# jorgeMFS/VCFX

Hardware: AMD Instinct MI355X
Metric: variant-records/sec (and GB/s vs HBM roofline), 427K var × 2504 samp (higher is better)
Workload: dtype u8; 1 GPU; VCFX_allele_freq_calc -i (file path) on a device-resident 427409 x 2504 VCF shard per GPU: the walk (line ends + allele counts + rows composed in LDS) + the rows in file order; records_per_gpu=427409, samples=2504, bytes_per_gpu=4297544426, parallelism=record-sharded x1

## Files before the change

### vcfx_amd/csrc/gpu/vcfxg_af_walk.hip

```cpp
#include <algorithm>
#include <type_traits>

#include "vcfxg_device.h"
#include "vcfxg_gt.h"
#include "vcfxg_kernels.h"
#include "vcfxg_walk.h"

namespace vcfxg {

#ifndef VCFXG_WALK_UNROLL
#define VCFXG_WALK_UNROLL 6
#endif
constexpr int kWalkUnroll = VCFXG_WALK_UNROLL;
#ifndef VCFXG_HWE_UNROLL
#define VCFXG_HWE_UNROLL 5
#endif
constexpr int kHweUnroll = VCFXG_HWE_UNROLL;
#ifndef VCFXG_GF_FLAGS
#define VCFXG_GF_FLAGS 1
#endif
constexpr bool kGfFlags = VCFXG_GF_FLAGS != 0;
#ifndef VCFXG_GF_UNROLL
#define VCFXG_GF_UNROLL 4
#endif
constexpr int kGfUnroll = VCFXG_GF_UNROLL;
#ifndef VCFXG_AF_XREC
#define VCFXG_AF_XREC 0
#endif
#ifndef VCFXG_AF_EXPT
#define VCFXG_AF_EXPT 0
#endif
#ifndef VCFXG_AF_EARLY
#define VCFXG_AF_EARLY 0
#endif
#define VCFXG_STR2(x) #x
#define VCFXG_STR(x) VCFXG_STR2(x)

template <class Op>
struct WalkRed;
template <>
struct WalkRed<AfOp> {
    static constexpr bool kAux = false;
    __device__ static AfOp make(const char *buf, int64_t ae) { return AfOp{buf, ae, 0}; }
    __device__ static void out(const AfOp &op, uint32_t &a, uint32_t &b, uint32_t &) {
        a = op.alt;
        b = op.tot;
    }
};
template <>
struct WalkRed<HweOp> {
    static constexpr bool kAux = true;
    __device__ static HweOp make(const char *buf, int64_t ae) { return HweOp{buf, ae}; }
    __device__ static void out(const HweOp &op, uint32_t &a, uint32_t &b, uint32_t &c) {
        a = op.c0;
        b = op.c1;
        c = op.c2;
    }
};

template <>
struct WalkRed<DoseWalkOp> {
    static constexpr bool kAux = false;
    __device__ static DoseWalkOp make(const char *buf, int64_t ae) { return DoseWalkOp{buf, ae}; }
    __device__ static void out(const DoseWalkOp &op, uint32_t &a, uint32_t &b, uint32_t &) {
        a = op.ns;
        b = op.na;
    }
};

template <>
struct WalkRed<DoseHeadOp> : WalkRed<DoseWalkOp> {
    __device__ static DoseHeadOp make(const char *buf, int64_t ae) { return DoseHeadOp{{buf, ae}}; }
};

template <class Op, bool kGF = false>
__global__ __launch_bounds__(kWalkThreads)
#ifdef VCFXG_WALK_MAXW
__attribute__((amdgpu_waves_per_eu(1, VCFXG_WALK_MAXW)))
#else
#ifndef VCFXG_AF_MINW
#define VCFXG_AF_MINW 5
#endif
__attribute__((amdgpu_waves_per_eu(kGF ? 4 : VCFXG_AF_MINW)))
#endif
void k_af_walk(const char *__restrict__ buf, int64_t lo, int64_t hi, int64_t chunk, int64_t n_walkers, int mode,
               int64_t span0, uint64_t cap_w, uint64_t *__restrict__ le_o, int32_t *__restrict__ alt_o,
               int32_t *__restrict__ tot_o, int32_t *__restrict__ aux_o, uint32_t *__restrict__ rowpre_o,
               uint8_t *__restrict__ status_o, LineMeta *__restrict__ meta_o, uint64_t *__restrict__ wcount,
               uint32_t *__restrict__ wgt, unsigned *overflow, WalkTail tail) {
    typedef WalkRed<Op> R;
    __shared__ uint4 win[kWalkWaves][2][kWave];
    constexpr bool kStageLds = std::is_same<Op, AfOp>::value;
    constexpr uint32_t kStgCap = kStageLds ? 2048u : 16u;
    __shared__ __attribute__((aligned(16))) char stg[kStageLds ? kWalkWaves : 1][kStgCap];
    const int wv = threadIdx.x / kWave;
    const int64_t wk = uniform64((int64_t)walk_block() * kWalkWaves + wv);
    if (wk >= n_walkers) return;
    const int strip_cr = mode == 0 ? 1 : 0;
    const int64_t cs = lo + wk * chunk;
    const int64_t ce = std::min<int64_t>(cs + chunk, hi);
    int64_t L, ce2;
    walker_lines(buf, lo, hi, cs, ce, L, ce2, chunk);
    const int64_t L0 = L;
    uint64_t wtext = 0;
    int64_t span = span0;
    uint8_t cr_prev = 0;
    uint64_t n = 0;
    uint32_t ngt = 0, ngf = 0;
    bool dirty = false;
    const uint64_t base = (uint64_t)wk * cap_w;
    uint64_t r_le = 0, r_S = 0;
    uint32_t r_alt = 0, r_tot = 0, r_aux = 0, r_pre = 0, r_k = 0;
    uint32_t r_h = 0;
    auto flush = [&](uint64_t first, uint32_t cnt) {
        if ((uint32_t)lane() < cnt) {
            const uint64_t o = base + first + lane();
            const uint8_t kind = (uint8_t)r_k;
            LineMeta m{};
            m.kind = kind;
            m.cr = (uint8_t)(r_k >> 16);
            m.pad = (R::kAux || std::is_same<Op, DoseHeadOp>::value) ? (uint8_t)r_h : 0;
            if (kind == kMetaGt) {
                m.S = r_S;
                m.rowpre = r_pre;
                m.sep = (uint8_t)(r_k >> 8);
            }
            le_o[o] = r_le;
            alt_o[o] = (int32_t)r_alt;
            tot_o[o] = (int32_t)r_tot;
            if (R::kAux) aux_o[o] = (int32_t)r_aux;
            rowpre_o[o] = kind == kMetaGt ? r_pre : 0u;
            status_o[o] = (uint8_t)(r_k >> 24);
            meta_o[o] = m;
        }
    };
    constexpr bool kXrec = VCFXG_AF_XREC && std::is_same<Op, AfOp>::value && !kGF;
    uint4 xv[kXrec ? kWalkUnroll : 1];
    int64_t xvb = -1;
    int cur = 0;
    int64_t A = L & ~(int64_t)15;
    if (L < ce2) prefetch_window(buf, A, hi, win[wv][cur]);
    constexpr bool kEarly = VCFXG_AF_EARLY && std::is_same<Op, AfOp>::value && !kGF && !kXrec;
    uint4 ev[kEarly ? kWalkUnroll : 1];
    const int64_t hlast = (hi - 1) & ~(int64_t)15;
    while (L < ce2) {
        if (n >= cap_w) {
            if (lane() == 0) atomicOr(overflow, 1u);
            break;
        }
        if constexpr (kEarly) {
#pragma unroll
            for (int u = 0; u < kWalkUnroll; u++) {
                const int64_t g = A + u * kWaveStep + kBlockBytes * lane();
                ev[u] = load16(buf, g < hi ? g : hlast);
            }
        }
        int64_t eA = kEarly ? A : -1;
        const int Lr = (int)(L - A);
        const uint4 *cw = win[wv][cur];
        int hr, N1r, r4 = 0, r7 = 0, r8 = 0;
        uint32_t ntab, first, hflags = 0;
        auto take = [&](const int(&rt)[9], bool comma) {
            r4 = rt[4];
            r7 = rt[7];
            r8 = rt[8];
            if (R::kAux) {
                const bool empty = rt[0] == Lr || rt[1] == rt[0] + 1 || r4 == rt[3] + 1;
                hflags = (comma ? kHweAltComma : 0u) | (empty ? kHweEmptyField : 0u);
            }
        };
        uint32_t w4 = 0;
        bool long_head = false;
        {
            if constexpr (kEarly) asm volatile("s_waitcnt vmcnt(" VCFXG_STR(VCFXG_WALK_UNROLL) ")" ::: "memory");
            else asm volatile("s_waitcnt vmcnt(0)" ::: "memory");
            w4 = reinterpret_cast<const uint32_t *>(cw)[lane()];
            hr = (int)std::min<int64_t>(hi - A, kWin);
            const uint32_t rg = range4(Lr, hr);
            N1r = first_match<4>(zero_bytes(w4 ^ kRepNl) & rg);
            int rt[9] = {};
            ntab = first_tabs<4>(zero_bytes(w4 ^ kRepTab) & rg, N1r >= 0 ? N1r : hr, rt);
            first = dword_byte(w4, Lr);
            if (ntab >= 9) take(rt, R::kAux && __ballot((zero_bytes(w4 ^ 0x2C2C2C2Cu) & range4(rt[3] + 1, rt[4])) != 0u));
        }
        if (N1r < 0 && ntab < 9 && first != '#' && hr == kWin) {
            prefetch_window(buf, A, hi, win[wv][cur], kWaveStep);
            long_head = true;
            const uint4 W = read_window(cw);
            const int b = 16 * lane();
            hr = (int)std::min<int64_t>(hi - A, kWaveStep);
            N1r = first_match<16>(eq_mask16(W, kRepNl) & range16(b, Lr, hr));
            int rt[9] = {};
            ntab = first_tabs<16>(eq_mask16(W, kRepTab) & range16(b, Lr, hr), N1r >= 0 ? N1r : hr, rt);
            if (ntab >= 9) take(rt, R::kAux && __ballot((eq_mask16(W, 0x2C2C2C2Cu) & range16(b, rt[3] + 1, rt[4])) != 0u));
        }
        auto wbyte = [&](int o) { return long_head ? slot_byte(cw, o) : dword_byte(w4, o); };
        const int64_t wend = A + hr;
        int64_t t4 = -1, t8 = -1;
        bool gt_head = false, gt_only = false;
        if (ntab >= 9 && first != '#') {
            t4 = A + r4;
            t8 = A + r8;
            if (r8 - r7 >= 3 && wbyte(r7 + 1) == 'G' && wbyte(r7 + 2) == 'T') {
                gt_only = r8 - r7 == 3;
                gt_head = gt_only || wbyte(r7 + 3) == ':';
            }
        }
        int64_t E;
        uint8_t cr = 0;
        bool predicted = false;
        const bool gf = kGF && N1r < 0 && gt_head && !gt_only;
        if (N1r >= 0) {
            E = A + N1r;
            cr = strip_cr && E > L && wbyte(N1r - 1) == '\r';
        } else if (gf) {
            E = hi;
        } else if (gt_only && span > 0 && t8 + 1 + span <= hi) {
            E = t8 + 1 + span;
            cr = cr_prev;
            predicted = true;
        } else {
            E = scan_nl(buf, wend, hi);
            cr = strip_cr && E > L && __builtin_amdgcn_readfirstlane(byte_at(buf, E - 1)) == '\r';
        }
        const uint32_t sep_w = gt_head && t8 + 2 < wend ? wbyte((int)(t8 + 2 - A)) : 0u;
        const int nxt = cur ^ 1;
        int64_t An = std::max<int64_t>(E - 1, 0) & ~(int64_t)15;
        bool pending = true;
        auto pre = [&]() {
            prefetch_window(buf, An, hi, win[wv][nxt]);
            pending = false;
        };
        uint8_t st = 0, kind = 0, sep = 0;
        uint32_t alt = 0, tot = 0, aux = 0, rowpre = 0;
        int64_t S = 0;
        bool ok = false;
        bool skip = std::is_same<Op, DoseHeadOp>::value && predicted;
        int64_t xuse = xvb;
        xvb = -1;
        auto sweep = [&]() {
            if constexpr (kGF) {
              if (gf) {
                S = t8 + 1;
                Op op = R::make(buf, hi);
                int64_t Eo = hi;
                uint8_t cro = 0;
                auto pre_e = [&](int64_t e) {
                    An = std::max<int64_t>(e - 1, 0) & ~(int64_t)15;
                    pre();
                };
                if constexpr (std::is_same<Op, AfOp>::value && kGfFlags)
                    ok = gt_first_af<kGfUnroll>(buf, S, hi, strip_cr, op, pre_e, Eo, cro);
                else
                    ok = gt_first<kWalkUnroll>(buf, S, hi, strip_cr, op, pre_e, Eo, cro);
                E = Eo;
                cr = cro;
                const int64_t ae = E - cr;
                kind = t8 < ae ? kMetaGt : kMetaFull;
                ok = ok && kind == kMetaGt;
                if (kind == kMetaGt) {
                    rowpre = (uint32_t)(t4 - L + 1);
                    sep = t8 + 2 >= ae ? 0
                          : t8 + 2 < wend ? (uint8_t)sep_w
                                          : (uint8_t)__builtin_amdgcn_readfirstlane(byte_at(buf, t8 + 2));
                    R::out(op, alt, tot, aux);
                }
                return;
              }
            }
            const int64_t ae = E - cr;
            if (ae <= L) kind = kMetaEmpty;
            else if (first == '#') kind = kMetaHeader;
            else if (gt_head && t8 < ae) kind = kMetaGt;
            else kind = kMetaFull;
            ok = false;
            if (kind == kMetaGt) {
                S = t8 + 1;
                rowpre = (uint32_t)(t4 - L + 1);
                sep = t8 + 2 >= ae ? 0
                      : t8 + 2 < wend ? (uint8_t)sep_w
                                      : (uint8_t)__builtin_amdgcn_readfirstlane(byte_at(buf, t8 + 2));
                Op op = R::make(buf, ae);
                if constexpr (kXrec) {
                    const int64_t use = xuse >= 0 && xuse <= S ? xuse : -1;
                    xuse = -1;
                    const int64_t nb = E + 1 < ce2 ? (E + 1) & ~(int64_t)15 : -1;
                    int64_t vbo;
                    ok = af_fixed_x<kWalkUnroll>(buf, S, ae, hi, op, sep, pre, xv, use, nb, vbo);
                    xvb = vbo;
                } else if constexpr (kEarly) {
                    const bool mine = eA >= 0 && eA <= S;
                    ok = af_fixed<kWalkUnroll>(buf, S, ae, op, sep, pre, mine ? ev : nullptr, mine ? eA : -1);
                    eA = -1;
                } else if constexpr (std::is_same<Op, AfOp>::value)
                    ok = af_fixed < kGF ? kGfUnroll : kWalkUnroll > (buf, S, ae, op, sep, pre);
                else if constexpr (std::is_same<Op, DoseHeadOp>::value) {
                    if (skip) {
                        ok = (sep == '/' || sep == '|') && ae - S >= 3 && ((ae - S + 1) & 3) == 0;
                        op.ns = ok ? (uint32_t)((ae - S + 1) >> 2) : 0u;
                        op.na = 0;
                    } else {
                        ok = gt_fast<kWalkUnroll>(buf, S, ae, op, sep, pre);
                    }
                } else ok = gt_fast < std::is_same<Op, HweOp>::value ? kHweUnroll : kWalkUnroll > (buf, S, ae, op, sep, pre);
                R::out(op, alt, tot, aux);
            }
        };
        sweep();
        if (pending) pre();
        if (predicted) {
            const uint4 *nw = win[wv][nxt];
            asm volatile("s_waitcnt vmcnt(0)" ::: "memory");
            const uint32_t be = slot_byte(nw, (int)(E - An)), be1 = slot_byte(nw, (int)(E - 1 - An));
            const bool endok = (E < hi ? be == '\n' : true) && ((strip_cr && be1 == '\r') == (cr != 0));
            if (!(ok && endok)) {
                const int64_t Et = scan_nl(buf, wend, hi);
                if (Et != E || !endok) {
                    skip = false;
                    E = Et;
                    cr = strip_cr && E > L && __builtin_amdgcn_readfirstlane(byte_at(buf, E - 1)) == '\r';
                    An = std::max<int64_t>(E - 1, 0) & ~(int64_t)15;
                    pending = true;
                    sweep();
                    if (pending) pre();
                }
            }
        }
        if constexpr (std::is_same<Op, DoseHeadOp>::value)
            if (skip && kind == kMetaGt) hflags |= kWalkUnswept;
        if (kind == kMetaGt) {
            if (ok) {
                st = 1;
                span = E - S;
                cr_prev = cr;
            } else {
                st = kAfPending;
            }
        }
        if ((uint32_t)lane() == (uint32_t)(n & 63)) {
            r_le = (uint64_t)E;
            r_S = (uint64_t)S;
            r_alt = alt;
            r_tot = tot;
            r_aux = aux;
            r_h = hflags;
            r_pre = rowpre;
            r_k = (uint32_t)kind | ((uint32_t)sep << 8) | ((uint32_t)cr << 16) | ((uint32_t)st << 24);
        }
        if constexpr (std::is_same<Op, AfOp>::value) {
            if (tail.stage && !(VCFXG_AF_EXPT & 1)) {
                if (kind == kMetaGt && ok && wtext + rowpre + 7u <= std::min<uint32_t>(tail.stage_cap, kStgCap)) {
                    uint32_t flo = 0x30303030u, fhi = 0x0A3030u;
                    if (!(VCFXG_AF_EXPT & 2)) af_freq_text(mode, (int32_t)alt, (int32_t)tot, flo, fhi);
                    auto *dst = reinterpret_cast<__attribute__((address_space(3))) char *>(
                                    reinterpret_cast<__attribute__((address_space(3))) char *>(
                                        (__attribute__((address_space(3))) void *)stg[kStageLds ? wv : 0])) +
                                wtext;
                    const unsigned char *src = reinterpret_cast<const unsigned char *>(cw) + (L - A);
                    for (uint32_t j0 = 0; j0 < rowpre + 7u; j0 += kWave) {
                        const uint32_t j = j0 + (uint32_t)lane();
                        if (j < rowpre) dst[j] = (char)src[j];
                        else if (j < rowpre + 7u) {
                            const uint32_t q = j - rowpre;
                            dst[j] = (char)((q < 4u ? flo >> (8u * q) : fhi >> (8u * (q - 4u))) & 0xFFu);
                        }
                    }
                } else if (kind == kMetaGt || kind == kMetaFull) {
                    dirty = true;
                }
            }
        }
        ngt += kind == kMetaGt ? 1u : 0u;
        if constexpr (kGF) ngf += gf && kind == kMetaGt && ok ? 1u : 0u;
        if (tail.wtext) {
            if (kind == kMetaGt) wtext += (uint64_t)rowpre + 7u;
            if (kind == kMetaFull || (kind == kMetaGt && !ok)) {
                if (lane() == 0) {
                    const unsigned long long e = atomicAdd(tail.cx_n, 1ull);
                    if (e < tail.cx_cap) tail.cx_list[e] = base + n;
                }
            }
        }
        n++;
        if ((n & 63) == 0) flush(n - 64, 64);
        L = E + 1;
        A = An;
        cur = nxt;
    }
    if (n & 63) flush(n & ~(uint64_t)63, (uint32_t)(n & 63));
    if constexpr (kStageLds) {
        if (tail.stage && wtext) {
            __builtin_amdgcn_fence(__ATOMIC_RELEASE, "wavefront");
            __builtin_amdgcn_wave_barrier();
            __builtin_amdgcn_fence(__ATOMIC_ACQUIRE, "wavefront");
            const uint32_t wt = (uint32_t)std::min<uint64_t>(wtext, kStgCap);
            char *gs = tail.stage + (uint64_t)wk * tail.stage_cap;
            for (uint32_t o = (uint32_t)lane() * 16u; o < wt; o += kWave * 16u)
                *reinterpret_cast<uint4 *>(gs + o) = *reinterpret_cast<const uint4 *>(stg[wv] + o);
        }
    }
    if (lane() == 0) {
        wcount[wk] = n;
        if (tail.wtext) {
            tail.wtext[wk] = wtext;
            tail.wstart[wk] = (uint64_t)L0;
        }
        wgt[wk] = ngt | (ngf << 16);
        if (tail.wdirty) tail.wdirty[wk] = dirty || n >= cap_w ? 1 : 0;
    }
}

#ifndef VCFXG_COMPACT_SUB
#define VCFXG_COMPACT_SUB 4
#endif
constexpr int kCompactSub = VCFXG_COMPACT_SUB, kCompactLanes = kWave / kCompactSub;
__global__ __launch_bounds__(256) void k_walk_compact(int64_t n_walkers, uint64_t cap_w,
                                                      const uint64_t *__restrict__ offs,
                                                      const uint32_t *__restrict__ wgt,
                                                      const uint64_t *__restrict__ le_b,
                                                      const int32_t *__restrict__ alt_b,
                                                      const int32_t *__restrict__ tot_b,
                                                      const int32_t *__restrict__ aux_b,
                                                      const uint32_t *__restrict__ rowpre_b,
                                                      const uint8_t *__restrict__ status_b,
                                                      const LineMeta *__restrict__ meta_b, uint64_t *line_end,
                                                      int32_t *alt, int32_t *tot, int32_t *aux, uint32_t *rowpre,
                                                      uint8_t *status, LineMeta *meta, uint64_t *n_lines,
                                                      unsigned long long *counters, const uint64_t *__restrict__ bpre) {
    __shared__ uint32_t red[256 / kWave];
    uint32_t g = 0;
    const int64_t nwaves = (int64_t)gridDim.x * (256 / kWave);
    const int sub = lane() / kCompactLanes, sl = lane() % kCompactLanes;
    for (int64_t w0 = ((int64_t)blockIdx.x * (256 / kWave) + threadIdx.x / kWave) * kCompactSub; w0 < n_walkers;
         w0 += nwaves * kCompactSub) {
        const int64_t w = w0 + sub;
        if (w >= n_walkers) continue;
        const uint64_t d0 = offs[w] + (bpre ? bpre[w / kWalkerScanBlock] : 0),
                       cnt = offs[w + 1] + (bpre ? bpre[(w + 1) / kWalkerScanBlock] : 0) - d0, s0 = (uint64_t)w * cap_w;
        g += sl == 0 ? (wgt[w] & 0xFFFFu) : 0u;
        for (uint64_t i = sl; i < cnt; i += kCompactLanes) {
            const uint64_t sl = s0 + i, d = d0 + i;
            line_end[d] = le_b[sl];
            alt[d] = alt_b[sl];
            tot[d] = tot_b[sl];
            if (aux_b) aux[d] = aux_b[sl];
            rowpre[d] = rowpre_b[sl];
            status[d] = status_b[sl];
            meta[d] = meta_b[sl];
        }
    }
    g = wave_sum(g);
    if (lane() == 0) red[threadIdx.x / kWave] = g;
    __syncthreads();
    if (threadIdx.x == 0) {
        uint32_t t = 0;
        for (int k = 0; k < 256 / kWave; k++) t += red[k];
        if (t) {
            atomicAdd(&counters[0], (unsigned long long)t);
            atomicAdd(&counters[1], (unsigned long long)t);
        }
        if (blockIdx.x == 0) *n_lines = offs[n_walkers] + (bpre ? bpre[n_walkers / kWalkerScanBlock] : 0);
    }
}

int64_t af_walkers(int64_t lo, int64_t hi, int64_t chunk) { return hi > lo ? (hi - lo + chunk - 1) / chunk : 0; }

hipError_t launch_af_walk(const char *buf, int64_t lo, int64_t hi, int64_t chunk, int mode, int64_t span0,
                          uint64_t cap_w, uint64_t *le_b, int32_t *alt_b, int32_t *tot_b, uint32_t *rowpre_b,
                          uint8_t *status_b, void *meta_b, uint64_t *wcount, uint32_t *wgt, unsigned *overflow,
                          hipStream_t s, int32_t *hwe_aux_b, const WalkTail *tail, bool dose, bool gt_first_walk,
                          bool dose_head) {
    const WalkTail t = tail ? *tail : WalkTail{};
    const int64_t nw = af_walkers(lo, hi, chunk);
    if (!nw) return hipErrorInvalidValue;
    const unsigned grid = (unsigned)((nw + kWalkWaves - 1) / kWalkWaves);
    if (gt_first_walk)
        hipLaunchKernelGGL(HIP_KERNEL_NAME(k_af_walk<AfOp, true>), dim3(grid), dim3(kWalkThreads), 0, s, buf, lo, hi,
                           chunk, nw, mode, span0, cap_w, le_b, alt_b, tot_b, nullptr, rowpre_b, status_b,
                           static_cast<LineMeta *>(meta_b), wcount, wgt, overflow, t);
    else if (dose && dose_head)
        hipLaunchKernelGGL(k_af_walk<DoseHeadOp>, dim3(grid), dim3(kWalkThreads), 0, s, buf, lo, hi, chunk, nw, mode,
                           span0, cap_w, le_b, alt_b, tot_b, nullptr, rowpre_b, status_b, static_cast<LineMeta *>(meta_b),
                           wcount, wgt, overflow, t);
    else if (dose)
        hipLaunchKernelGGL(k_af_walk<DoseWalkOp>, dim3(grid), dim3(kWalkThreads), 0, s, buf, lo, hi, chunk, nw, mode,
                           span0, cap_w, le_b, alt_b, tot_b, nullptr, rowpre_b, status_b, static_cast<LineMeta *>(meta_b),
                           wcount, wgt, overflow, t);
    else if (hwe_aux_b)
        hipLaunchKernelGGL(k_af_walk<HweOp>, dim3(grid), dim3(kWalkThreads), 0, s, buf, lo, hi, chunk, nw, mode, span0,
                           cap_w, le_b, alt_b, tot_b, hwe_aux_b, rowpre_b, status_b, static_cast<LineMeta *>(meta_b),
                           wcount, wgt, overflow, t);
    else
        hipLaunchKernelGGL(k_af_walk<AfOp>, dim3(grid), dim3(kWalkThreads), 0, s, buf, lo, hi, chunk, nw, mode, span0,
                           cap_w, le_b, alt_b, tot_b, nullptr, rowpre_b, status_b, static_cast<LineMeta *>(meta_b),
                           wcount, wgt, overflow, t);
    return hipGetLastError();
}

hipError_t launch_walk_compact(int64_t n_walkers, uint64_t cap_w, const uint64_t *offs, const uint32_t *wgt,
                               const uint64_t *le_b, const int32_t *alt_b, const int32_t *tot_b,
                               const uint32_t *rowpre_b, const uint8_t *status_b, const void *meta_b,
                               uint64_t *line_end, int32_t *alt, int32_t *tot, uint32_t *rowpre, uint8_t *status,
                               void *meta, uint64_t *n_lines, unsigned long long *counters, hipStream_t s,
                               const int32_t *aux_b, int32_t *aux, const uint64_t *bpre) {
    const int64_t blocks = std::min<int64_t>((n_walkers + 256 / kWave - 1) / (256 / kWave), 512);
    hipLaunchKernelGGL(k_walk_compact, dim3((unsigned)std::max<int64_t>(blocks, 1)), dim3(256), 0, s, n_walkers, cap_w,
                       offs, wgt, le_b, alt_b, tot_b, aux_b, rowpre_b, status_b, static_cast<const LineMeta *>(meta_b),
                       line_end, alt, tot, aux, rowpre, status, static_cast<LineMeta *>(meta), n_lines, counters, bpre);
    return hipGetLastError();
}

}
```

### vcfx_amd/csrc/gpu/vcfxg_gt.h

```cpp
#pragma once
#include <algorithm>
#include <type_traits>

#include "vcfxg_device.h"

#ifndef VCFXG_AF_ROLL
#define VCFXG_AF_ROLL 0
#endif
#ifndef VCFXG_GF_BUF
#define VCFXG_GF_BUF 1
#endif

#ifndef VCFXG_FQ_EXPT
#define VCFXG_FQ_EXPT 0
#endif

namespace vcfxg {

struct DwordView {
    uint32_t d;
    uint32_t f;
    uint32_t dig;
    bool real;
    int64_t p;
};

template <class Op>
__device__ __forceinline__ void fast_dword(uint32_t d, uint32_t exp_xor, uint32_t &err, Op &op, bool real,
                                           int64_t p) {
    uint32_t e = d ^ exp_xor;
    err |= e & 0xFF00FF00u;
    uint32_t f = e & 0x00FF00FFu;
    uint32_t notdig = (f + 0x00F600F6u) & 0x01000100u;
    uint32_t notdot = ((f ^ 0x001E001Eu) + 0x00FF00FFu) & 0x01000100u;
    err |= notdig & notdot;
    DwordView v{d, f, notdig ^ 0x01000100u, real, p};
    op.dword(v);
}

#ifndef VCFXG_UNROLL
#define VCFXG_UNROLL 4
#endif
#ifndef VCFXG_NT_SWEEP
#define VCFXG_NT_SWEEP 0
#endif
struct NoPre {
    __device__ void operator()() const {}
};
template <class T, class = void>
struct HasClean : std::false_type {};
template <class T>
struct HasClean<T, std::void_t<decltype(&T::clean)>> : std::true_type {};
template <class T, class = void>
struct HasCleanAt : std::false_type {};
template <class T>
struct HasCleanAt<T, std::void_t<decltype(&T::clean_at)>> : std::true_type {};
template <int kUnroll = VCFXG_UNROLL, class Op, class Pre = NoPre>
__device__ bool gt_fast(const char *__restrict__ buf, int64_t S, int64_t E, Op &op, uint32_t sep_hint = 0,
                        Pre pre = Pre(), int64_t *swept = nullptr) {
    S = uniform64(S);
    E = uniform64(E);
    int64_t L = E - S;
    if (L < 3 || ((L + 1) & 3)) return false;
    uint32_t sepc = sep_hint ? sep_hint : byte_at(buf, S + 1);
    sepc = __builtin_amdgcn_readfirstlane(sepc);
    if (sepc != '/' && sepc != '|') return false;
    const uint32_t exp_xor = 0x09000000u | (sepc << 8) | 0x00300030u;
    const uint32_t neutral = 0x092E002Eu | (sepc << 8);
    op.begin(sepc, neutral);
    const int s = (int)(S & 3);
    const int64_t b0 = S & ~(int64_t)15;
    const char *__restrict__ base = buf + b0;
    const int Sr = (int)(S - b0), Er = (int)(E - b0);
#if VCFXG_NT_SWEEP
    const int lastblk = (Er - 1) & ~15;
#endif
    uint32_t err = 0;
    if (swept) *swept = E;
    const int lo16 = lane() * kBlockBytes;
#if !VCFXG_NT_SWEEP
    const __amdgpu_buffer_rsrc_t rs = buf_rsrc(base, (uint32_t)((Er + 15) & ~15));
#endif
    for (int w0 = 0; w0 < Er; w0 += kUnroll * kWaveStep) {
        uint4 v[kUnroll];
        uint32_t x4[kUnroll];
#pragma unroll
        for (int u = 0; u < kUnroll; u++) {
            const int blk = w0 + u * kWaveStep + lo16;
#if VCFXG_NT_SWEEP
            const int bl = blk < Er ? blk : lastblk;
            {
                typedef unsigned int v4u __attribute__((ext_vector_type(4)));
                const v4u t = __builtin_nontemporal_load(reinterpret_cast<const v4u *>(base + bl));
                v[u] = make_uint4(t.x, t.y, t.z, t.w);
            }
            x4[u] = load4(base, bl + 16);
#else
            v[u] = bload16(rs, blk);
            x4[u] = bload4(rs, blk + 16);
#endif
        }
        if (w0 == 0) pre();
#pragma unroll
        for (int u = 0; u < kUnroll; u++) {
            const int w = w0 + u * kWaveStep;
            const int blk = w + lo16;
            const bool interior = (w + s >= Sr) && (w + kWaveStep - 1 + s < Er);
            if (blk < Er) {
                uint32_t d[4] = {__builtin_amdgcn_alignbyte(v[u].y, v[u].x, s),
                                 __builtin_amdgcn_alignbyte(v[u].z, v[u].y, s),
                                 __builtin_amdgcn_alignbyte(v[u].w, v[u].z, s),
                                 __builtin_amdgcn_alignbyte(x4[u], v[u].w, s)};
                bool clean = false;
                if constexpr (HasClean<Op>::value || HasCleanAt<Op>::value) {
                    if (interior) {
                        const uint32_t e0 = d[0] ^ exp_xor, e1 = d[1] ^ exp_xor, e2 = d[2] ^ exp_xor,
                                       e3 = d[3] ^ exp_xor;
                        clean = !__any(((e0 | e1 | e2 | e3) & ~0x00010001u) != 0u);
                        if (clean) {
                            if constexpr (HasCleanAt<Op>::value) op.clean_at(e0, e1, e2, e3, b0 + blk + s);
                            else op.clean(e0, e1, e2, e3);
                        }
                    }
                }
                bool real[4] = {true, true, true, true};
                if (!interior) {
                    const int q0 = blk + s - Sr, last = Er - Sr - 3;
#pragma unroll
                    for (int i = 0; i < 4; i++) {
                        const int q = q0 + 4 * i;
                        if (q < 0 || q > last) {
                            d[i] = neutral;
                            real[i] = false;
                        } else if (q == last) d[i] = (d[i] & 0x00FFFFFFu) | 0x09000000u;
                    }
                }
                if (!clean) {
#pragma unroll
                    for (int i = 0; i < 4; i++) fast_dword(d[i], exp_xor, err, op, real[i], b0 + blk + s + 4 * i);
                }
            }
        }
        if (op.done()) {
            if (swept && b0 + w0 + kUnroll * kWaveStep < E) *swept = b0 + w0 + kUnroll * kWaveStep;
            break;
        }
        if (__any(err != 0u)) return false;
    }
    if (__any(err != 0u)) return false;
    op.finish();
    return true;
}

template <class Op>
__device__ void gt_general(const char *__restrict__ buf, int64_t S, int64_t E, Op &op) {
    for (int64_t w = S & ~(int64_t)15; w < E; w += kWaveStep) {
        int64_t blk = w + (int64_t)lane() * kBlockBytes;
        if (blk < E) {
            uint32_t tm = eq_mask16(load16(buf, blk), kRepTab);
            uint32_t starts = (tm << 1) & 0xFFFFu;
            if (blk > 0 && byte_at(buf, blk - 1) == '\t') starts |= 1u;
            starts &= range_mask16(blk, S + 1, E);
            if (S >= blk && S < blk + 16) starts |= 1u << (S - blk);
            while (starts) {
                int j = __builtin_ctz(starts);
                starts &= starts - 1u;
                op.sample(blk + j);
            }
        }
        if (op.done()) break;
    }
    op.finish();
}

__device__ __forceinline__ int64_t sample_end(const char *__restrict__ buf, int64_t st, int64_t E) {
    int64_t p = st;
    while (p < E && byte_at(buf, p) != '\t') p++;
    return p;
}

__device__ __forceinline__ bool gt_special(uint32_t c) {
    return c == '/' || c == '|' || c == ':' || c == '\t' || c == ' ' || c == '\r';
}
template <int kU, class Op, class Pre>
__device__ bool gt_first(const char *__restrict__ buf, int64_t S, int64_t hi, int strip_cr, Op &op, Pre pre,
                         int64_t &E_out, uint8_t &cr_out) {
    S = uniform64(S);
    int64_t E = hi, ae = hi;
    bool found = false, bad = false;
    uint32_t carry = 0;
    const int64_t b0 = S & ~(int64_t)15;
    const int lo16 = lane() * kBlockBytes;
    for (int64_t w0 = b0; w0 < hi && !found; w0 += kU * kWaveStep) {
        uint4 v[kU];
        uint32_t x4[kU];
#pragma unroll
        for (int u = 0; u < kU; u++) {
            const int64_t blk = w0 + u * kWaveStep + lo16;
            const int64_t bl = blk < hi ? blk : ((hi - 1) & ~(int64_t)15);
            v[u] = load16(buf, bl);
            x4[u] = load4(buf, bl + 16);
        }
#pragma unroll
        for (int u = 0; u < kU; u++) {
            if (found) break;
            const int64_t blk = w0 + u * kWaveStep + lo16;
            const uint32_t nlm = blk < hi ? eq_mask16(v[u], kRepNl) & range_mask16(blk, S, hi) : 0u;
            const uint64_t anyn = __ballot(nlm != 0u);
            if (anyn) {
                const int k = __builtin_ctzll(anyn);
                E = uniform64(w0 + u * kWaveStep + 16 * k + __builtin_ctz((uint32_t)__shfl((int)nlm, k)));
                found = true;
                const uint32_t cr = strip_cr && E > S ? __builtin_amdgcn_readfirstlane(byte_at(buf, E - 1)) == '\r' : 0u;
                cr_out = (uint8_t)cr;
                ae = E - cr;
                pre(E);
            }
            const uint32_t tm = eq_mask16(v[u], kRepTab);
            const uint32_t last = lane_prev(v[u].w >> 24);
            const uint32_t prev = lane() ? last : carry;
            carry = lane_last(v[u].w >> 24);
            uint32_t starts = ((tm << 1) & 0xFFFFu) | (prev == '\t' ? 1u : 0u);
            if (S >= blk && S < blk + 16) starts |= 1u << (S - blk);
            starts &= range_mask16(blk, S, ae);
            const uint32_t wd[5] = {v[u].x, v[u].y, v[u].z, v[u].w, x4[u]};
            while (starts) {
                const int o = __builtin_ctz(starts);
                starts &= starts - 1u;
                const int q = o >> 2;
                const uint32_t lo = q == 0 ? wd[0] : q == 1 ? wd[1] : q == 2 ? wd[2] : wd[3];
                const uint32_t hw = q == 0 ? wd[1] : q == 1 ? wd[2] : q == 2 ? wd[3] : wd[4];
                const uint32_t d = __builtin_amdgcn_alignbyte(hw, lo, (uint32_t)(o & 3));
                const uint32_t c0 = d & 0xFFu, c1 = (d >> 8) & 0xFFu, c2 = (d >> 16) & 0xFFu, c3 = d >> 24;
                const int64_t p3 = blk + o + 3;
                const bool quick = (c1 == '/' || c1 == '|') && !gt_special(c0) && !gt_special(c2) &&
                                   (p3 == ae || (p3 < ae && (c3 == ':' || c3 == '\t')));
                if (quick) op.gt3(c0, c2);
                else bad = true;
            }
        }
    }
    if (!found) {
        E = hi;
        const uint32_t cr = strip_cr && E > S ? __builtin_amdgcn_readfirstlane(byte_at(buf, E - 1)) == '\r' : 0u;
        cr_out = (uint8_t)cr;
        pre(E);
    }
    E_out = E;
    if (__any(bad)) return false;
    op.finish();
    return true;
}
struct NoPreE {
    __device__ void operator()(int64_t) const {}
};
template <int kU = 8, class Op>
__device__ __forceinline__ bool gt_first_known(const char *__restrict__ buf, int64_t S, int64_t ae, Op &op) {
    int64_t e;
    uint8_t cr;
    return gt_first<kU>(buf, S, ae, 0, op, NoPreE(), e, cr);
}

struct AfOp {
    const char *buf;
    int64_t E;
    int gi;
    uint32_t alt = 0, tot = 0;
    __device__ void begin(uint32_t, uint32_t) {}
    __device__ bool done() const { return false; }
    __device__ void dword(const DwordView &v) {
        tot += __popc(v.dig);
        alt += __popc((v.f + 0x00FF00FFu) & v.dig);
    }
    __device__ void gt3(uint32_t c0, uint32_t c2) {
        tot += (c0 - '0' < 10u) + (c2 - '0' < 10u);
        alt += (c0 - '1' < 9u) + (c2 - '1' < 9u);
    }
    __device__ void sample(int64_t st) {
        int64_t p = st;
        for (int k = 0; k < gi; k++) {
            while (p < E) {
                uint32_t c = byte_at(buf, p);
                if (c == '\t' || c == ':') break;
                p++;
            }
            if (p >= E || byte_at(buf, p) == '\t') return;
            p++;
        }
        bool in_tok = false, first_dot = false, numeric = true, nonzero = false;
        for (;; p++) {
            uint32_t c = p < E ? byte_at(buf, p) : (uint32_t)'\t';
            bool end = (c == '\t' || c == ':');
            if (end || c == '/' || c == '|') {
                if (in_tok && !first_dot && numeric) {
                    tot++;
                    if (nonzero) alt++;
                }
                in_tok = false;
                if (end) break;
                continue;
            }
            if (!in_tok) {
                in_tok = true;
                first_dot = (c == '.');
                numeric = true;
                nonzero = false;
            }
            if (c < '0' || c > '9') numeric = false;
            else if (c != '0') nonzero = true;
        }
    }
    __device__ void finish() {
        alt = wave_sum(alt);
        tot = wave_sum(tot);
    }
};

__device__ __forceinline__ uint32_t fixed4_mmap(double v) {
    double sc = __dadd_rn(__dmul_rn(v, 10000.0), 0.5);
    return (uint32_t)(unsigned long long)sc;
}
__device__ __forceinline__ uint32_t fixed4_printf(double v) {
    if (v == 0.0) return 0u;
    uint64_t bits = __double_as_longlong(v);
    int ex = (int)((bits >> 52) & 0x7FF);
    uint64_t m = bits & ((1ull << 52) - 1);
    int q;
    if (ex == 0) q = 1074;
    else { m |= 1ull << 52; q = 1075 - ex; }
    if (q <= 0) return 10000u * (uint32_t)(m << -q);
    unsigned __int128 num = (unsigned __int128)m * 10000u;
    if (q >= 100) return 0u;
    unsigned __int128 k = num >> q;
    unsigned __int128 rem = num - (k << q);
    unsigned __int128 half = (unsigned __int128)1 << (q - 1);
    if (rem > half || (rem == half && (k & 1))) k += 1;
    return (uint32_t)k;
}

__device__ __forceinline__ void af_freq_text(int mode, int32_t a, int32_t t, uint32_t &lo, uint32_t &hi) {
    const double f = t > 0 ? __ddiv_rn((double)a, (double)t) : 0.0;
    const uint32_t k4 = mode == 0 ? fixed4_mmap(f) : fixed4_printf(f);
    const uint32_t ip = k4 / 10000u, fp = k4 % 10000u;
    lo = ('0' + ip) | ((uint32_t)'.' << 8) | (('0' + fp / 1000u) << 16) | (('0' + (fp / 100u) % 10u) << 24);
    hi = ('0' + (fp / 10u) % 10u) | (('0' + fp % 10u) << 8) | ((uint32_t)'\n' << 16);
}
template <int kU, class Pre>
__device__ bool gt_first_af(const char *__restrict__ buf, int64_t S, int64_t hi, int strip_cr, AfOp &op, Pre pre,
                            int64_t &E_out, uint8_t &cr_out) {
    S = uniform64(S);
    constexpr uint32_t M = 0x80808080u, K = 0x7F7F7F7Fu;
    int64_t E = hi, ae = hi;
    bool found = false;
    uint32_t bad = 0, asc = 0, tot = 0, alt = 0;
    uint32_t carry = 0;
    uint32_t scarry = 0;
    const int64_t b0 = S & ~(int64_t)15;
    const int lo16 = lane() * kBlockBytes;
    const int64_t hend = (hi + 15) & ~(int64_t)15;
    for (int64_t w0 = b0; w0 < hi && !found; w0 += kU * kWaveStep) {
        uint4 v[kU];
        uint32_t x4[kU];
#if VCFXG_GF_BUF
        const __amdgpu_buffer_rsrc_t rs =
            buf_rsrc(buf + w0, (uint32_t)std::min<int64_t>(hend - w0, (int64_t)kU * kWaveStep + 16));
#pragma unroll
        for (int u = 0; u < kU; u++) {
            v[u] = bload16(rs, u * kWaveStep + lo16);
            x4[u] = bload4(rs, u * kWaveStep + lo16 + 16);
        }
#else
#pragma unroll
        for (int u = 0; u < kU; u++) {
            const int64_t blk = w0 + u * kWaveStep + lo16;
            const int64_t bl = blk < hi ? blk : hend - 16;
            v[u] = load16(buf, bl);
            x4[u] = load4(buf, bl + 16);
        }
#endif
#pragma unroll
        for (int u = 0; u < kU; u++) {
            if (found) break;
            const int64_t ws = w0 + u * kWaveStep, blk = ws + lo16;
            const uint32_t W[5] = {v[u].x, v[u].y, v[u].z, v[u].w, x4[u]};
            const uint32_t wor = W[0] | W[1] | W[2] | W[3];
            asc |= wor | W[4];
            const bool first = ws == b0, edge = first || ws + kWaveStep > hi;
            uint32_t nlm = 0;
            if (edge) nlm = blk < hi ? eq_mask16(v[u], kRepNl) & range_mask16(blk, S, hi) : 0u;
            else
                nlm = (~(((W[0] ^ kRepNl) + K) & ((W[1] ^ kRepNl) + K) & ((W[2] ^ kRepNl) + K) &
                         ((W[3] ^ kRepNl) + K)) | wor) & M;
            uint64_t anyn = __ballot(nlm != 0u);
            if (anyn && !edge) {
                nlm = eq_mask16(v[u], kRepNl);
                anyn = __ballot(nlm != 0u);
            }
            if (anyn) {
                const int k = __builtin_ctzll(anyn);
                E = uniform64(ws + 16 * k + __builtin_ctz((uint32_t)__shfl((int)nlm, k)));
                found = true;
                const uint32_t cr = strip_cr && E > S ? __builtin_amdgcn_readfirstlane(byte_at(buf, E - 1)) == '\r' : 0u;
                cr_out = (uint8_t)cr;
                ae = E - cr;
                pre(E);
            }
            const uint32_t tab3 = ~((W[3] ^ kRepTab) + K);
            const uint32_t up = lane_prev(tab3);
            uint32_t tprev = lane() ? up : carry;
            carry = lane_last(tab3);
            uint32_t rm = 0xFFFFu;
            if (edge || found) {
                rm = blk < hi ? range_mask16(blk, S, ae) : 0u;
                rm |= ((S >= blk && S < blk + 16) ? 1u << (S - blk) : 0u) << 16;
            }
            uint32_t st[4];
            {
                uint32_t tp = tprev;
#pragma unroll
                for (int i = 0; i < 4; i++) {
                    const uint32_t tb = i == 3 ? tab3 : ~((W[i] ^ kRepTab) + K);
                    uint32_t x = __builtin_amdgcn_alignbyte(tb, tp, 3) & M;
                    if (edge || found)
                        x = (x | nib_bytes((rm >> (16 + 4 * i)) & 0xFu)) & nib_bytes((rm >> (4 * i)) & 0xFu) & M;
                    st[i] = x;
                    tp = tb;
                }
            }
            const uint32_t sup = lane_prev(st[3]);
            const uint32_t sprev = lane() ? sup : scarry;
            scarry = lane_last(st[3]);
            auto classes = [&](uint32_t x, uint32_t &sep, uint32_t &trm, uint32_t &vv, uint32_t &dg, uint32_t &nz) {
                const uint32_t nt = (x ^ kRepTab) + K, nn = (x ^ kRepNl) + K, nc = (x ^ kRepColon) + K;
                trm = ~(nt & nn & nc);
                const uint32_t ns = (x ^ 0x2F2F2F2Fu) + K;
                sep = ~(ns & ((x ^ 0x7C7C7C7Cu) + K));
                const uint32_t g9 = x + 0x46464646u;
                dg = (x + 0x50505050u) & ~g9;
                nz = (x + 0x4F4F4F4Fu) & ~g9;
                vv = (x + 0x52525252u) & ~g9 & ns;
            };
            uint32_t sep0, trm0, v0, dg0, nz0;
            classes(W[0], sep0, trm0, v0, dg0, nz0);
#pragma unroll
            for (int i = 0; i < 4; i++) {
                uint32_t sep1, trm1, v1, dg1, nz1;
                classes(W[i + 1], sep1, trm1, v1, dg1, nz1);
                const uint32_t s1 = __builtin_amdgcn_alignbyte(sep1, sep0, 1);
                const uint32_t c3 = __builtin_amdgcn_alignbyte(trm1, trm0, 3);
                const uint32_t s2 = __builtin_amdgcn_alignbyte(st[i], i ? st[i - 1] : sprev, 2);
                const uint32_t u = st[i] | s2;
                bad |= (st[i] & ~(s1 & c3)) | (u & ~v0);
                tot = popc_acc(u & dg0, tot);
                alt = popc_acc(u & nz0, alt);
                sep0 = sep1, trm0 = trm1, v0 = v1, dg0 = dg1, nz0 = nz1;
            }
        }
    }
    if (!found) {
        E = hi;
        const uint32_t cr = strip_cr && E > S ? __builtin_amdgcn_readfirstlane(byte_at(buf, E - 1)) == '\r' : 0u;
        cr_out = (uint8_t)cr;
        pre(E);
    }
    E_out = E;
    if (__any((bad | (asc & M)) != 0u)) return false;
    op.alt = wave_sum32(alt);
    op.tot = wave_sum32(tot);
    return true;
}

template <int kUnroll, class Pre>
__device__ bool af_fixed(const char *__restrict__ buf, int64_t S, int64_t E, AfOp &op, uint32_t sep_hint, Pre pre,
                         const uint4 *first = nullptr, int64_t vb = -1) {
    S = uniform64(S);
    E = uniform64(E);
    const int64_t L = E - S;
    if (L < 3 || ((L + 1) & 3)) return false;
    uint32_t sepc = sep_hint ? sep_hint : byte_at(buf, S + 1);
    sepc = __builtin_amdgcn_readfirstlane(sepc);
    if (sepc != '/' && sepc != '|') return false;
    const uint32_t sh = 8u * (uint32_t)(S & 3);
    auto rot = [&](uint32_t x) { return sh ? (x << sh) | (x >> (32u - sh)) : x; };
    const uint32_t exp = rot(0x09300030u | (sepc << 8));
    const uint32_t mbin = rot(0xFFFEFFFEu);
    const uint32_t msep = rot(0xFF00FF00u);
    const uint32_t fsh = (S & 1) ? 8u : 0u;
    const int64_t b0 = vb >= 0 ? uniform64(vb) : S & ~(int64_t)15;
    const char *__restrict__ base = buf + b0;
    const int Sr = (int)(S - b0), Er = (int)(E - b0);
    const __amdgpu_buffer_rsrc_t rs = buf_rsrc(base, (uint32_t)((Er + 15) & ~15));
    const int lo16 = lane() * kBlockBytes;
    uint32_t alt = 0, dots = 0, err = 0, alt8 = 0;
    static_assert(4 * kUnroll <= 255, "af_fixed: bytewise allele sums");
#if VCFXG_AF_ROLL
    uint4 v[kUnroll];
#pragma unroll
    for (int u = 0; u < kUnroll; u++) v[u] = bload16(rs, u * kWaveStep + lo16);
    pre();
#endif
    for (int w0 = 0; w0 < Er; w0 += kUnroll * kWaveStep) {
#if !VCFXG_AF_ROLL
        uint4 v[kUnroll];
#pragma unroll
        for (int u = 0; u < kUnroll; u++) v[u] = first && w0 == 0 ? first[u] : bload16(rs, w0 + u * kWaveStep + lo16);
        if (w0 == 0) pre();
#endif
#if VCFXG_AF_ROLL
        const int wn = w0 + kUnroll * kWaveStep;
#endif
        auto dwords = [&](int u, const uint4 &x, uint32_t(&d)[4]) {
            d[0] = x.x, d[1] = x.y, d[2] = x.z, d[3] = x.w;
            const int w = w0 + u * kWaveStep;
            if (!(w >= Sr && w + kWaveStep <= Er)) {
                const int blk = w + lo16;
                const uint32_t rm = blk < Er ? range16(blk, Sr, Er) : 0u;
#pragma unroll
                for (int i = 0; i < 4; i++) {
                    const uint32_t bm = nib_bytes((rm >> (4 * i)) & 0xFu);
                    d[i] = (d[i] & bm) | (exp & ~bm);
                }
            }
        };
#pragma unroll
        for (int u = 0; u < kUnroll; u++) {
            uint32_t d[4];
            dwords(u, v[u], d);
#if VCFXG_AF_ROLL
            if (wn < Er) v[u] = bload16(rs, wn + u * kWaveStep + lo16);
#endif
            const uint32_t e0 = d[0] ^ exp, e1 = d[1] ^ exp, e2 = d[2] ^ exp, e3 = d[3] ^ exp;
            const uint32_t berr = (e0 | e1 | e2 | e3) & mbin;
            if (!__any(berr != 0u)) {
                alt8 += e0 + e1 + e2 + e3;
                continue;
            }
#pragma unroll
            for (int i = 0; i < 4; i++) {
                const uint32_t e = d[i] ^ exp;
                err |= e & msep;
                const uint32_t f = (e >> fsh) & 0x00FF00FFu;
                const uint32_t notdig = (f + 0x00F600F6u) & 0x01000100u;
                const uint32_t notdot = ((f ^ 0x001E001Eu) + 0x00FF00FFu) & 0x01000100u;
                err |= notdig & notdot;
                dots += __popc(notdig);
                alt += __popc((f + 0x00FF00FFu) & (notdig ^ 0x01000100u));
            }
        }
        if (__any(err != 0u)) return false;
        alt = __builtin_amdgcn_sad_u8(alt8, 0u, alt);
        alt8 = 0;
    }
    op.alt = wave_sum32(alt);
    op.tot = (uint32_t)(2 * ((L + 1) >> 2)) - wave_sum32(dots);
    return true;
}

template <int kUnroll, class Pre>
__device__ bool af_fixed_x(const char *__restrict__ buf, int64_t S, int64_t E, int64_t hi, AfOp &op, uint32_t sep_hint,
                           Pre pre, uint4 (&v)[kUnroll], int64_t vb, int64_t nb, int64_t &vb_out) {
    S = uniform64(S);
    E = uniform64(E);
    vb_out = -1;
    const int64_t L = E - S;
    if (L < 3 || ((L + 1) & 3)) return false;
    uint32_t sepc = sep_hint ? sep_hint : byte_at(buf, S + 1);
    sepc = __builtin_amdgcn_readfirstlane(sepc);
    if (sepc != '/' && sepc != '|') return false;
    const uint32_t sh = 8u * (uint32_t)(S & 3);
    auto rot = [&](uint32_t x) { return sh ? (x << sh) | (x >> (32u - sh)) : x; };
    const uint32_t exp = rot(0x09300030u | (sepc << 8));
    const uint32_t mbin = rot(0xFFFEFFFEu);
    const uint32_t msep = rot(0xFF00FF00u);
    const uint32_t fsh = (S & 1) ? 8u : 0u;
    const int64_t b0 = vb >= 0 ? uniform64(vb) : S & ~(int64_t)15;
    const char *__restrict__ base = buf + b0;
    const int Sr = (int)(S - b0), Er = (int)(E - b0);
    const int lastblk = (Er - 1) & ~15;
    const int lo16 = lane() * kBlockBytes;
    const int64_t hlast = (hi - 1) & ~(int64_t)15;
    uint32_t alt = 0, dots = 0, err = 0;
    if (vb < 0) {
#pragma unroll
        for (int u = 0; u < kUnroll; u++) {
            const int blk = u * kWaveStep + lo16;
            v[u] = load16(base, blk < Er ? blk : lastblk);
        }
    }
    pre();
    for (int w0 = 0; w0 < Er; w0 += kUnroll * kWaveStep) {
        const int wn = w0 + kUnroll * kWaveStep;
        auto dwords = [&](int u, const uint4 &x, uint32_t(&d)[4]) {
            d[0] = x.x, d[1] = x.y, d[2] = x.z, d[3] = x.w;
            const int w = w0 + u * kWaveStep;
            if (!(w >= Sr && w + kWaveStep <= Er)) {
                const int blk = w + lo16;
                const uint32_t rm = blk < Er ? range16(blk, Sr, Er) : 0u;
#pragma unroll
                for (int i = 0; i < 4; i++) {
                    const uint32_t bm = nib_bytes((rm >> (4 * i)) & 0xFu);
                    d[i] = (d[i] & bm) | (exp & ~bm);
                }
            }
        };
#pragma unroll
        for (int u = 0; u < kUnroll; u++) {
            uint32_t d[4];
            dwords(u, v[u], d);
            if (wn < Er) {
                const int blk = wn + u * kWaveStep + lo16;
                v[u] = load16(base, blk < Er ? blk : lastblk);
            } else if (nb >= 0) {
                const int64_t g = nb + u * kWaveStep + lo16;
                v[u] = load16(buf, g < hi ? g : hlast);
            }
            uint32_t berr = 0, balt = 0;
#pragma unroll
            for (int i = 0; i < 4; i++) {
                const uint32_t e = d[i] ^ exp;
                berr |= e & mbin;
                balt += __popc(e);
            }
            if (!__any(berr != 0u)) {
                alt += balt;
                continue;
            }
#pragma unroll
            for (int i = 0; i < 4; i++) {
                const uint32_t e = d[i] ^ exp;
                err |= e & msep;
                const uint32_t f = (e >> fsh) & 0x00FF00FFu;
                const uint32_t notdig = (f + 0x00F600F6u) & 0x01000100u;
                const uint32_t notdot = ((f ^ 0x001E001Eu) + 0x00FF00FFu) & 0x01000100u;
                err |= notdig & notdot;
                dots += __popc(notdig);
                alt += __popc((f + 0x00FF00FFu) & (notdig ^ 0x01000100u));
            }
        }
        if (__any(err != 0u)) return false;
    }
    op.alt = wave_sum32(alt);
    op.tot = (uint32_t)(2 * ((L + 1) >> 2)) - wave_sum32(dots);
    vb_out = nb;
    return true;
}

struct GqQuery {
    const char *q;
    int qlen;
    int strict;
    int qa, qb;
};

__device__ __forceinline__ bool is_digit(uint32_t c) { return c - '0' < 10u; }

__device__ __forceinline__ bool parse_diploid(const char *__restrict__ buf, int64_t g, int64_t n, int &a1, int &a2) {
    int64_t sep = -1;
    for (int64_t i = 0; i < n; i++) {
        uint32_t c = byte_at(buf, g + i);
        if (c == '|' || c == '/') { sep = i; break; }
    }
    if (sep <= 0 || sep == n - 1) return false;
    if (sep == 1 && byte_at(buf, g) == '.') return false;
    uint32_t v = 0;
    for (int64_t i = 0; i < sep; i++) {
        uint32_t c = byte_at(buf, g + i);
        if (!is_digit(c)) return false;
        v = v * 10u + (c - '0');
    }
    a1 = (int)v;
    if (n - sep - 1 == 1 && byte_at(buf, g + sep + 1) == '.') return false;
    v = 0;
    for (int64_t i = sep + 1; i < n; i++) {
        uint32_t c = byte_at(buf, g + i);
        if (!is_digit(c)) return false;
        v = v * 10u + (c - '0');
    }
    a2 = (int)v;
    return true;
}

__device__ __forceinline__ bool gt_matches(const char *__restrict__ buf, int64_t g, int64_t n, const GqQuery &Q) {
    if (Q.strict) {
        if (n != Q.qlen) return false;
        for (int64_t i = 0; i < n; i++)
            if (byte_at(buf, g + i) != (uint32_t)(uint8_t)Q.q[i]) return false;
        return true;
    }
    if (n == 3 && Q.qlen == 3) {
        uint32_t s = byte_at(buf, g + 1);
        if (s != '|' && s != '/') return false;
        uint32_t g0 = byte_at(buf, g), g1 = byte_at(buf, g + 2);
        if (!is_digit(g0) || !is_digit(g1)) return false;
        int ga = (int)(g0 - '0'), gb = (int)(g1 - '0');
        if (ga > gb) { int t = ga; ga = gb; gb = t; }
        return ga == Q.qa && gb == Q.qb;
    }
    int a1 = 0, a2 = 0;
    if (!parse_diploid(buf, g, n, a1, a2)) return false;
    if (a1 > a2) { int t = a1; a1 = a2; a2 = t; }
    return a1 == Q.qa && a2 == Q.qb;
}

struct GqOp {
    const char *buf;
    int64_t E;
    int gi;
    GqQuery Q;
    uint32_t p1 = 0, p2 = 0, pmask = 0;
    uint32_t mn = ~0u;
    bool any = false;
    bool found = false;
    __device__ void begin(uint32_t sepc, uint32_t) {
        begin_patterns();
        if (!pmask) p1 = p2 = ~0u;
        (void)sepc;
    }
    __device__ void begin_patterns() {
        if (Q.strict) {
            if (Q.qlen == 3) {
                p1 = p2 = (uint32_t)(uint8_t)Q.q[0] | ((uint32_t)(uint8_t)Q.q[1] << 8) | ((uint32_t)(uint8_t)Q.q[2] << 16);
                pmask = 0x00FFFFFFu;
            } else pmask = 0;
        } else if (Q.qa >= 0 && Q.qa <= 9 && Q.qb >= 0 && Q.qb <= 9) {
            p1 = (uint32_t)('0' + Q.qa) | ((uint32_t)('0' + Q.qb) << 16);
            p2 = (uint32_t)('0' + Q.qb) | ((uint32_t)('0' + Q.qa) << 16);
            pmask = 0x00FF00FFu;
        } else pmask = 0;
    }
    __device__ bool done() {
        return (VCFXG_FQ_EXPT & 1) ? false : (found = found || __any(any || mn == 0u));
    }
    __device__ void dword(const DwordView &v) {
        const uint32_t x = (v.d & pmask) | (v.real ? 0u : 0x01000000u);
        mn = std::min(mn, std::min(x ^ p1, x ^ p2));
    }
    __device__ void sample(int64_t st) {
        if (any) return;
        int64_t se = sample_end(buf, st, E);
        int64_t p = st, fs = st;
        int fi = 0;
        for (;; p++) {
            bool end = (p == se) || byte_at(buf, p) == ':';
            if (end) {
                if (fi == gi) break;
                fi++;
                fs = p + 1;
                if (p == se) return;
            }
        }
        int64_t n = p - fs;
        if (n > 0 && gt_matches(buf, fs, n, Q)) any = true;
    }
    __device__ void finish() { found = __any(any || mn == 0u); }
};

struct NrOp {
    const char *buf;
    int64_t E;
    int gi, mode;
    bool any = false;
    bool found = false;
    __device__ void begin(uint32_t, uint32_t) {}
    __device__ bool done() { return found = found || __any(any); }
    __device__ void dword(const DwordView &v) { any = any || (v.real && v.f != 0u); }
    __device__ void sample(int64_t st) {
        if (any) return;
        const int64_t se = sample_end(buf, st, E);
        int64_t p = st, fs = st;
        int fi = 0;
        for (;; p++) {
            const bool end = (p == se) || byte_at(buf, p) == ':';
            if (end) {
                if (fi == gi) break;
                fi++;
                fs = p + 1;
                if (p == se) {
                    any = true;
                    return;
                }
            }
        }
        const int64_t n = p - fs;
        bool hr = n > 0;
        bool only = n > 0;
        for (int64_t k = fs; only && k < p; k++) {
            const uint32_t c = byte_at(buf, k);
            only = c == '0' || c == '/' || c == '|';
        }
        if (n == 3) {
            const uint32_t c1 = byte_at(buf, fs + 1);
            const bool pat = byte_at(buf, fs) == '0' && (c1 == '/' || c1 == '|') && byte_at(buf, fs + 2) == '0';
            hr = pat || (mode == 1 && only);
        } else hr = only;
        if (!hr) any = true;
    }
    __device__ void finish() { found = __any(any); }
};

struct MdOp {
    bool any = false;
    bool found = false;
    __device__ void begin(uint32_t, uint32_t) {}
    __device__ bool done() { return found = found || __any(any); }
    __device__ void dword(const DwordView &v) { any = any || (v.real && v.dig != 0x01000100u); }
    __device__ void finish() { found = __any(any); }
};

__device__ __forceinline__ int hwe_parse(const char *__restrict__ buf, int64_t p, int64_t end) {
    if (p >= end) return -1;
    for (int64_t k = p; k < end; k++)
        if (byte_at(buf, k) == ':') {
            end = k;
            break;
        }
    while (p < end && (byte_at(buf, p) == ' ' || byte_at(buf, p) == '\r')) p++;
    if (p >= end || !is_digit(byte_at(buf, p))) return -1;
    uint32_t a1 = 0, a2 = 0;
    while (p < end && is_digit(byte_at(buf, p))) {
        a1 = a1 * 10u + (byte_at(buf, p) - '0');
        p++;
    }
    if (p >= end || (byte_at(buf, p) != '/' && byte_at(buf, p) != '|')) return -1;
    p++;
    if (p >= end || !is_digit(byte_at(buf, p))) return -1;
    while (p < end && is_digit(byte_at(buf, p))) {
        a2 = a2 * 10u + (byte_at(buf, p) - '0');
        p++;
    }
    if ((int32_t)a1 > 1 || (int32_t)a2 > 1) return -1;
    if (a1 == 0u && a2 == 0u) return 0;
    if (a1 == 1u && a2 == 1u) return 2;
    return 1;
}

struct DoseWalkOp {
    const char *buf;
    int64_t E;
    uint32_t ns = 0, na = 0;
    __device__ void begin(uint32_t, uint32_t) {}
    __device__ bool done() const { return false; }
    __device__ void dword(const DwordView &v) {
        ns += v.real;
        na += v.real && v.dig != 0x01000100u;
    }
    __device__ void finish() {
        ns = wave_sum(ns);
        na = wave_sum(na);
    }
};

struct DoseHeadOp : DoseWalkOp {};

struct HweOp {
    const char *buf;
    int64_t E;
    uint32_t c0 = 0, c1 = 0, c2 = 0;
    uint32_t nv_alt = 0, two = 0;
    __device__ void begin(uint32_t, uint32_t) {}
    __device__ bool done() const { return false; }
    __device__ void dword(const DwordView &v) {
        const bool ok = (v.f & 0x00FE00FEu) == 0u;
        nv_alt += ok ? (uint32_t)__popc(v.f) + 0x10000u : 0u;
        two += v.f == 0x00010001u;
    }
    __device__ void clean(uint32_t e0, uint32_t e1, uint32_t e2, uint32_t e3) {
        nv_alt = popc_acc(e3, popc_acc(e2, popc_acc(e1, popc_acc(e0, nv_alt + 0x40000u))));
        two += (e0 & (e0 >> 16)) + (e1 & (e1 >> 16)) + (e2 & (e2 >> 16)) + (e3 & (e3 >> 16));
    }
    __device__ void gt3(uint32_t c0, uint32_t c2) {
        const bool ok = (c0 - '0' < 2u) && (c2 - '0' < 2u);
        const uint32_t s = (c0 - '0') + (c2 - '0');
        c0_ += ok && s == 0u;
        c1_ += ok && s == 1u;
        c2_ += ok && s == 2u;
    }
    uint32_t c0_ = 0, c1_ = 0, c2_ = 0;
    __device__ void sample(int64_t st) {
        const int g = hwe_parse(buf, st, sample_end(buf, st, E));
        c0 += g == 0;
        c1 += g == 1;
        c2 += g == 2;
    }
    __device__ void finish() {
        const uint32_t nv = nv_alt >> 16, alt = nv_alt & 0xFFFFu;
        c2 += two + c2_;
        c1 += alt - 2u * two + c1_;
        c0 += nv - (alt - two) + c0_;
        c0 = wave_sum(c0);
        c1 = wave_sum(c1);
        c2 = wave_sum(c2);
    }
};

}
```

Measured before the change: 488.4 million records/s.

## Stage per-record walk results in an LDS ring instead of per-lane registers

```diff
diff --git a/vcfx_amd/csrc/gpu/vcfxg_af_walk.hip b/vcfx_amd/csrc/gpu/vcfxg_af_walk.hip
--- a/vcfx_amd/csrc/gpu/vcfxg_af_walk.hip
+++ b/vcfx_amd/csrc/gpu/vcfxg_af_walk.hip
@@ -93,6 +93,9 @@
     constexpr bool kStageLds = std::is_same<Op, AfOp>::value;
     constexpr uint32_t kStgCap = kStageLds ? 2048u : 16u;
     __shared__ __attribute__((aligned(16))) char stg[kStageLds ? kWalkWaves : 1][kStgCap];
+    constexpr bool kEntX = R::kAux || std::is_same<Op, DoseHeadOp>::value;
+    constexpr int kEnt = kEntX ? 10 : 8;
+    __shared__ __attribute__((aligned(16))) uint32_t ring[kWalkWaves][kWave * kEnt];
     const int wv = threadIdx.x / kWave;
     const int64_t wk = uniform64((int64_t)walk_block() * kWalkWaves + wv);
     if (wk >= n_walkers) return;
@@ -109,17 +112,22 @@
     uint32_t ngt = 0, ngf = 0;
     bool dirty = false;
     const uint64_t base = (uint64_t)wk * cap_w;
-    uint64_t r_le = 0, r_S = 0;
-    uint32_t r_alt = 0, r_tot = 0, r_aux = 0, r_pre = 0, r_k = 0;
-    uint32_t r_h = 0;
+    uint32_t *const rg = ring[wv];
     auto flush = [&](uint64_t first, uint32_t cnt) {
+        __builtin_amdgcn_fence(__ATOMIC_RELEASE, "wavefront");
+        __builtin_amdgcn_wave_barrier();
+        __builtin_amdgcn_fence(__ATOMIC_ACQUIRE, "wavefront");
         if ((uint32_t)lane() < cnt) {
+            const uint32_t *e = rg + (uint32_t)lane() * kEnt;
+            const uint64_t r_le = (uint64_t)e[0] | ((uint64_t)e[1] << 32), r_S = (uint64_t)e[2] | ((uint64_t)e[3] << 32);
+            const uint32_t r_alt = e[4], r_tot = e[5], r_pre = e[6], r_k = e[7];
+            const uint32_t r_aux = kEntX ? e[kEnt - 2] : 0u, r_h = kEntX ? e[kEnt - 1] : 0u;
             const uint64_t o = base + first + lane();
             const uint8_t kind = (uint8_t)r_k;
             LineMeta m{};
             m.kind = kind;
             m.cr = (uint8_t)(r_k >> 16);
-            m.pad = (R::kAux || std::is_same<Op, DoseHeadOp>::value) ? (uint8_t)r_h : 0;
+            m.pad = kEntX ? (uint8_t)r_h : 0;
             if (kind == kMetaGt) {
                 m.S = r_S;
                 m.rowpre = r_pre;
@@ -133,6 +141,8 @@
             status_o[o] = (uint8_t)(r_k >> 24);
             meta_o[o] = m;
         }
+        __builtin_amdgcn_fence(__ATOMIC_RELEASE, "wavefront");
+        __builtin_amdgcn_wave_barrier();
     };
     constexpr bool kXrec = VCFXG_AF_XREC && std::is_same<Op, AfOp>::value && !kGF;
     uint4 xv[kXrec ? kWalkUnroll : 1];
@@ -337,15 +347,24 @@
                 st = kAfPending;
             }
         }
-        if ((uint32_t)lane() == (uint32_t)(n & 63)) {
-            r_le = (uint64_t)E;
-            r_S = (uint64_t)S;
-            r_alt = alt;
-            r_tot = tot;
-            r_aux = aux;
-            r_h = hflags;
-            r_pre = rowpre;
-            r_k = (uint32_t)kind | ((uint32_t)sep << 8) | ((uint32_t)cr << 16) | ((uint32_t)st << 24);
+        {
+            uint32_t ent = 0;
+#define VCFXG_PUT(j, x) \
+    asm("v_writelane_b32 %0, %1, " #j : "+v"(ent) : "s"(__builtin_amdgcn_readfirstlane((uint32_t)(x))))
+            VCFXG_PUT(0, (uint32_t)E);
+            VCFXG_PUT(1, (uint64_t)E >> 32);
+            VCFXG_PUT(2, (uint32_t)S);
+            VCFXG_PUT(3, (uint64_t)S >> 32);
+            VCFXG_PUT(4, alt);
+            VCFXG_PUT(5, tot);
+            VCFXG_PUT(6, rowpre);
+            VCFXG_PUT(7, (uint32_t)kind | ((uint32_t)sep << 8) | ((uint32_t)cr << 16) | ((uint32_t)st << 24));
+            if constexpr (kEntX) {
+                VCFXG_PUT(8, aux);
+                VCFXG_PUT(9, hflags);
+            }
+#undef VCFXG_PUT
+            if (lane() < kEnt) rg[(uint32_t)(n & 63) * kEnt + (uint32_t)lane()] = ent;
         }
         if constexpr (std::is_same<Op, AfOp>::value) {
             if (tail.stage && !(VCFXG_AF_EXPT & 1)) {
diff --git a/vcfx_amd/csrc/gpu/vcfxg_gt.h b/vcfx_amd/csrc/gpu/vcfxg_gt.h
--- a/vcfx_amd/csrc/gpu/vcfxg_gt.h
+++ b/vcfx_amd/csrc/gpu/vcfxg_gt.h
@@ -489,11 +489,11 @@
     const int64_t b0 = vb >= 0 ? uniform64(vb) : S & ~(int64_t)15;
     const char *__restrict__ base = buf + b0;
     const int Sr = (int)(S - b0), Er = (int)(E - b0);
-    const __amdgpu_buffer_rsrc_t rs = buf_rsrc(base, (uint32_t)((Er + 15) & ~15));
     const int lo16 = lane() * kBlockBytes;
     uint32_t alt = 0, dots = 0, err = 0, alt8 = 0;
     static_assert(4 * kUnroll <= 255, "af_fixed: bytewise allele sums");
 #if VCFXG_AF_ROLL
+    const __amdgpu_buffer_rsrc_t rs = buf_rsrc(base, (uint32_t)((Er + 15) & ~15));
     uint4 v[kUnroll];
 #pragma unroll
     for (int u = 0; u < kUnroll; u++) v[u] = bload16(rs, u * kWaveStep + lo16);
@@ -501,9 +501,12 @@
 #endif
     for (int w0 = 0; w0 < Er; w0 += kUnroll * kWaveStep) {
 #if !VCFXG_AF_ROLL
+        const __amdgpu_buffer_rsrc_t rb = buf_rsrc(base + w0, (uint32_t)(((Er + 15) & ~15) - w0));
+        int lo = lo16;
+        asm("" : "+v"(lo));
         uint4 v[kUnroll];
 #pragma unroll
-        for (int u = 0; u < kUnroll; u++) v[u] = first && w0 == 0 ? first[u] : bload16(rs, w0 + u * kWaveStep + lo16);
+        for (int u = 0; u < kUnroll; u++) v[u] = first && w0 == 0 ? first[u] : bload16(rb, u * kWaveStep + lo);
         if (w0 == 0) pre();
 #endif
 #if VCFXG_AF_ROLL
```

Result: no change. 488.7 million records/s (median of 6 runs) (+0.1%).
